# microsoft/SpeechT5

Measured on NVIDIA H100. Metric: utterances/sec (TTS fine-tune step, 10s@16kHz), higher is better.
Workload: dtype bf16

## Files before the change

### speecht5_b200/csrc/attention_flash.cu

```cuda
#include "../../include/speecht5_b200.h"
#include "kernels.cuh"
#include "ptx.cuh"
#include "tma_map.cuh"

namespace st5 {

int set_error(int code, const char* where);

constexpr int FL_T = 64;
constexpr int FL_THREADS = 9 * 32;
constexpr int FL_PE_ROWS = 128;
constexpr int FL_SP = FL_T + 4;
constexpr int FL_QPP = FL_PE_ROWS + 4;
constexpr int FL_MAX_TK_RESIDENT = 320;
constexpr int FL_MAX_T_RPE_RESIDENT = 160;
template <bool RPE> constexpr size_t fl_smem() {
  return 8192 + 2 * 8192 + 8192 + 8192 + 2 * (size_t)FL_T * FL_SP * 4 +
         (RPE ? 2 * 16384 + (size_t)FL_T * FL_QPP * 4 : 0) + 128 + 512 + 1024;
}

struct FlashFwdParams {
  int B, H, Tq, Tk, causal, maxpos;
  float scale_log2;
  const uint8_t* key_pad;
  __nv_bfloat16* out; long o_ld, o_bs;
  float* out_f32;
  float* lse; float* inv_l;
  __nv_bfloat16* psave;
  void* probs; int probs_fp32; long p_ld;
  uint32_t drop_thr; float drop_scale; uint64_t seed, offset;
  int probs_heads;
};

__device__ __forceinline__ uint32_t fl_pack(float a, float b) {
  __nv_bfloat162 t = __floats2bfloat162_rn(a, b);
  return *reinterpret_cast<uint32_t*>(&t);
}
__host__ __device__ __forceinline__ int fl_window_row0(int i0, int j0, int maxpos) {
  int w = i0 - j0 - (FL_T - 1) + maxpos;
  const int hi = 2 * maxpos - FL_PE_ROWS;
  if (w > hi) w = hi;
  if (w < 0) w = 0;
  return w;
}
template <int NR>
__device__ __forceinline__ void fl_store_acc(float* dst, int pitch, const float (&d)[NR]) {
  const int l = (int)lane_id(), w = (threadIdx.x >> 5) & 3;
  const int r0 = 16 * w + (l >> 2);
#pragma unroll
  for (int i = 0; i < NR; i += 2) {
    const int r = r0 + 8 * ((i >> 1) & 1), c = 8 * (i >> 2) + 2 * (l & 3);
    *reinterpret_cast<float2*>(dst + r * pitch + c) = make_float2(d[i], d[i + 1]);
  }
}

template <bool RPE>
__global__ void __launch_bounds__(FL_THREADS, 1)
    attn_flash_fwd_kernel(const __grid_constant__ CUtensorMap map_q, const __grid_constant__ CUtensorMap map_k,
                          const __grid_constant__ CUtensorMap map_v, const __grid_constant__ CUtensorMap map_pe,
                          const FlashFwdParams p) {
  extern __shared__ __align__(1024) uint8_t smem_raw[];
  uint8_t* smem = reinterpret_cast<uint8_t*>((reinterpret_cast<uintptr_t>(smem_raw) + 1023) & ~uintptr_t(1023));
  uint8_t* sQ = smem;
  uint8_t* sK = sQ + 8192;
  uint8_t* sV = sK + 2 * 8192;
  uint8_t* sP = sV + 8192;
  float* sS = reinterpret_cast<float*>(sP + 8192);
  float* sO = sS + FL_T * FL_SP;
  uint8_t* sPE = reinterpret_cast<uint8_t*>(sO + FL_T * FL_SP);
  float* sQP = reinterpret_cast<float*>(sPE + (RPE ? 2 * 16384 : 0));
  uint64_t* bar_q = reinterpret_cast<uint64_t*>(reinterpret_cast<uint8_t*>(sQP) + (RPE ? FL_T * FL_QPP * 4 : 0));
  uint64_t* bar_k = bar_q + 1;
  uint64_t* bar_kfree = bar_q + 3;
  uint64_t* bar_s = bar_q + 5;
  uint64_t* bar_sfree = bar_q + 6;
  uint64_t* bar_v = bar_q + 7;
  uint64_t* bar_p = bar_q + 8;
  uint64_t* bar_pv = bar_q + 9;
  uint64_t* bar_o = bar_q + 10;
  float* red = reinterpret_cast<float*>(bar_q + 16);

  const int warp = threadIdx.x >> 5;
  const int nqt = (p.Tq + FL_T - 1) / FL_T;
  const int qt = nqt - 1 - (int)blockIdx.x;
  const int h = blockIdx.y, b = blockIdx.z;
  const int i0 = qt * FL_T;
  int tk = p.Tk;
  if (p.causal && i0 + FL_T < tk) tk = i0 + FL_T;
  const int nkb = (tk + FL_T - 1) / FL_T;
  void* const probs = (p.probs_heads > 0 && h >= p.probs_heads) ? nullptr : p.probs;
  const int nsweep = probs != nullptr ? 3 : 2;
  const int NS = nsweep * nkb;

  if (warp == 4 && elect_one()) {
    tma_prefetch_desc(&map_q);
    tma_prefetch_desc(&map_k);
    tma_prefetch_desc(&map_v);
    if constexpr (RPE) tma_prefetch_desc(&map_pe);
    mbar_init(bar_q, 1);
    for (int s = 0; s < 2; ++s) {
      mbar_init(&bar_k[s], 1);
      mbar_init(&bar_kfree[s], 1);
    }
    mbar_init(bar_s, 128);
    mbar_init(bar_sfree, 4);
    mbar_init(bar_v, 1);
    mbar_init(bar_p, 4);
    mbar_init(bar_pv, 1);
    mbar_init(bar_o, 128);
    fence_mbar_init();
  }
  __syncthreads();
  pdl_sync();

  if (warp == 4) {
    if (elect_one()) {
      mbar_expect_tx(bar_q, 8192);
      tma_load_4d(sQ, &map_q, bar_q, 0, i0, h, b);
      int pv = 0;
      for (int s = 0; s < NS; ++s) {
        const int sweep = s / nkb, kb = s - sweep * nkb;
        const int st = s & 1;
        if (s >= 2) mbar_wait_quiet(&bar_kfree[st], (uint32_t)(((s >> 1) - 1) & 1));
        mbar_expect_tx(&bar_k[st], 8192u + (RPE ? 16384u : 0u));
        tma_load_4d(sK + st * 8192, &map_k, &bar_k[st], 0, kb * FL_T, h, b);
        if constexpr (RPE)
          tma_load_4d(sPE + st * 16384, &map_pe, &bar_k[st], 0, fl_window_row0(i0, kb * FL_T, p.maxpos), 0, 0);
        if (sweep == 1) {
          if (pv > 0) mbar_wait_quiet(bar_pv, (uint32_t)((pv - 1) & 1));
          mbar_expect_tx(bar_v, 8192);
          tma_load_4d(sV, &map_v, bar_v, 0, kb * FL_T, h, b);
          ++pv;
        }
      }
    }
  } else if (warp < 4) {
    mbar_wait_quiet(bar_q, 0);
    const uint32_t aq = smem_u32(sQ), ap = smem_u32(sP), av = smem_u32(sV);
    float o[32];
#pragma unroll
    for (int t = 0; t < 32; ++t) o[t] = 0.f;
    int pv = 0;
    for (int s = 0; s < NS; ++s) {
      const int sweep = s / nkb;
      const int st = s & 1;
      mbar_wait_quiet(&bar_k[st], (uint32_t)((s >> 1) & 1));
      if (s > 0) mbar_wait_quiet(bar_sfree, (uint32_t)((s - 1) & 1));
      {
        float sc[32];
        const uint32_t ak = smem_u32(sK + st * 8192);
        wgmma_fence();
#pragma unroll
        for (int k = 0; k < 4; ++k)
          wgmma_m64n64<0, 0>(sc, wgmma_smem_desc(aq + k * 32, 16, 1024), wgmma_smem_desc(ak + k * 32, 16, 1024),
                             k != 0 ? 1u : 0u);
        wgmma_commit();
        if constexpr (RPE) {
          float qp[64];
          const uint32_t ape = smem_u32(sPE + st * 16384);
#pragma unroll
          for (int k = 0; k < 4; ++k)
            wgmma_m64n128<0, 0>(qp, wgmma_smem_desc(aq + k * 32, 16, 1024), wgmma_smem_desc(ape + k * 32, 16, 1024),
                                k != 0 ? 1u : 0u);
          wgmma_commit();
          wgmma_wait<0>();
          wgmma_fence_regs(qp);
          fl_store_acc(sQP, FL_QPP, qp);
        } else {
          wgmma_wait<0>();
        }
        wgmma_fence_regs(sc);
        if (threadIdx.x == 0) mbar_arrive(&bar_kfree[st]);
        fl_store_acc(sS, FL_SP, sc);
      }
      mbar_arrive(bar_s);
      if (sweep == 1) {
        mbar_wait_quiet(bar_v, (uint32_t)(pv & 1));
        mbar_wait_quiet(bar_p, (uint32_t)(pv & 1));
        wgmma_fence();
#pragma unroll
        for (int k = 0; k < 4; ++k)
          wgmma_m64n64<0, 1>(o, wgmma_smem_desc(ap + k * 32, 16, 1024), wgmma_smem_desc(av + k * 2048, 8192, 1024),
                             (pv | k) != 0 ? 1u : 0u);
        wgmma_commit();
        wgmma_wait<0>();
        wgmma_fence_regs(o);
        if (threadIdx.x == 0) mbar_arrive(bar_pv);
        ++pv;
      }
    }
    fl_store_acc(sO, FL_SP, o);
    mbar_arrive(bar_o);
  } else {
    const int sw = warp - 5;
    const int q = sw & 1;
    const int half = sw >> 1;
    const int lane = (int)lane_id();
    const int r = q * 32 + lane;
    const int i = i0 + r;
    const bool row_ok = i < p.Tq;
    const bool warp_live = i0 + q * 32 < p.Tq;
    const uint8_t* kp = p.key_pad != nullptr ? p.key_pad + (int64_t)b * p.Tk : nullptr;
    const int64_t prow = ((int64_t)b * p.H + h) * p.Tq + i;
    uint64_t dseed = p.seed, doffset = p.offset;
    if (p.drop_thr != 0) resolve_seed(dseed, doffset);
    float* probs_f = reinterpret_cast<float*>(probs);
    __nv_bfloat16* probs_h = reinterpret_cast<__nv_bfloat16*>(probs);

    float m = -INFINITY, mm = 0.f, sum = 0.f, inv = 0.f;
    int pv = 0;
    for (int sweep = 0; sweep < nsweep; ++sweep) {
      for (int kb = 0; kb < nkb; ++kb) {
        const int s = sweep * nkb + kb;
        const int j0 = kb * FL_T;
        mbar_wait_quiet(bar_s, (uint32_t)(s & 1));
        if (sweep == 1 && pv > 0) mbar_wait_quiet(bar_pv, (uint32_t)((pv - 1) & 1));
        const int c = half;
        const int jc = j0 + c * 32;
        const bool live = warp_live && jc < tk && !(p.causal && jc > i0 + q * 32 + 31);
        uint8_t* blk = sP + r * 128;
        const int cbase = c * 4;
        if (!live) {
          if (sweep == 1) {
#pragma unroll
            for (int g = 0; g < 4; ++g) {
              *reinterpret_cast<uint4*>(blk + (((cbase + g) ^ (r & 7)) << 4)) = make_uint4(0u, 0u, 0u, 0u);
              if (p.psave != nullptr && row_ok && jc + 8 * g + 8 <= p.p_ld)
                *reinterpret_cast<uint4*>(p.psave + prow * p.p_ld + jc + 8 * g) = make_uint4(0u, 0u, 0u, 0u);
            }
          } else if (sweep == 2 && row_ok) {
            for (int t = 0; t < 32; ++t)
              if (jc + t < p.p_ld) {
                if (p.probs_fp32) probs_f[prow * p.p_ld + jc + t] = 0.f;
                else probs_h[prow * p.p_ld + jc + t] = __float2bfloat16(0.f);
              }
          }
        } else {
          float v[32];
          {
            const float* src = sS + r * FL_SP + c * 32;
#pragma unroll
            for (int t = 0; t < 32; t += 4) {
              const float4 f = *reinterpret_cast<const float4*>(src + t);
              v[t] = f.x; v[t + 1] = f.y; v[t + 2] = f.z; v[t + 3] = f.w;
            }
          }
          uint32_t vb;
          {
            const int j = jc + lane;
            const bool ok = j < tk && !(kp != nullptr && kp[j] != 0);
            vb = __ballot_sync(0xffffffffu, ok);
            if (p.causal) {
              const int lim = i - jc;
              vb &= lim >= 31 ? 0xffffffffu : (lim < 0 ? 0u : ((2u << lim) - 1u));
            }
          }
          if constexpr (RPE) {
            const int w0 = fl_window_row0(i0, j0, p.maxpos);
            int colmax = 2 * p.maxpos - 1 - w0;
            if (colmax > FL_PE_ROWS - 1) colmax = FL_PE_ROWS - 1;
            const int off = i - jc + p.maxpos - w0;
            const float* qrow = sQP + r * FL_QPP;
#pragma unroll
            for (int t = 0; t < 32; ++t) {
              int col = off - t;
              col = col < 0 ? 0 : (col > colmax ? colmax : col);
              v[t] += qrow[col];
            }
          }
          if (sweep == 0) {
#pragma unroll
            for (int t = 0; t < 32; ++t)
              if ((vb >> t) & 1u) m = fmaxf(m, v[t] * p.scale_log2);
          } else if (sweep == 1) {
            uint32_t kb_ = 0xffffffffu;
            if (p.drop_thr != 0)
              kb_ = dropout_keep_mask32(dseed, doffset, (uint64_t)prow * attn_drop_pitch(p.Tk) + (uint64_t)jc, p.drop_thr);
            __nv_bfloat16* psv = (p.psave != nullptr && row_ok) ? p.psave + prow * p.p_ld + jc : nullptr;
#pragma unroll
            for (int g = 0; g < 4; ++g) {
              float ev[8];
#pragma unroll
              for (int t = 0; t < 8; ++t) {
                const int u = 8 * g + t;
                ev[t] = ((vb >> u) & 1u) ? fast_ex2(v[u] * p.scale_log2 - mm) : 0.f;
                sum += ev[t];
              }
              const uint32_t k8 = kb_ >> (8 * g);
              uint4 pk, ps;
              pk.x = fl_pack((k8 & 1u) ? ev[0] * p.drop_scale : 0.f, (k8 & 2u) ? ev[1] * p.drop_scale : 0.f);
              pk.y = fl_pack((k8 & 4u) ? ev[2] * p.drop_scale : 0.f, (k8 & 8u) ? ev[3] * p.drop_scale : 0.f);
              pk.z = fl_pack((k8 & 16u) ? ev[4] * p.drop_scale : 0.f, (k8 & 32u) ? ev[5] * p.drop_scale : 0.f);
              pk.w = fl_pack((k8 & 64u) ? ev[6] * p.drop_scale : 0.f, (k8 & 128u) ? ev[7] * p.drop_scale : 0.f);
              *reinterpret_cast<uint4*>(blk + (((cbase + g) ^ (r & 7)) << 4)) = pk;
              if (psv != nullptr && jc + 8 * g + 8 <= p.p_ld) {
                ps.x = fl_pack((k8 & 1u) ? ev[0] : -ev[0], (k8 & 2u) ? ev[1] : -ev[1]);
                ps.y = fl_pack((k8 & 4u) ? ev[2] : -ev[2], (k8 & 8u) ? ev[3] : -ev[3]);
                ps.z = fl_pack((k8 & 16u) ? ev[4] : -ev[4], (k8 & 32u) ? ev[5] : -ev[5]);
                ps.w = fl_pack((k8 & 64u) ? ev[6] : -ev[6], (k8 & 128u) ? ev[7] : -ev[7]);
                *reinterpret_cast<uint4*>(psv + 8 * g) = ps;
              }
            }
          } else if (row_ok) {
            if (p.probs_fp32) {
              float* dst = probs_f + prow * p.p_ld + jc;
              if (jc + 32 <= p.p_ld && (p.p_ld & 3) == 0) {
#pragma unroll
                for (int t = 0; t < 32; t += 4) {
                  float4 o4;
                  o4.x = ((vb >> t) & 1u) ? fast_ex2(v[t] * p.scale_log2 - mm) * inv : 0.f;
                  o4.y = ((vb >> (t + 1)) & 1u) ? fast_ex2(v[t + 1] * p.scale_log2 - mm) * inv : 0.f;
                  o4.z = ((vb >> (t + 2)) & 1u) ? fast_ex2(v[t + 2] * p.scale_log2 - mm) * inv : 0.f;
                  o4.w = ((vb >> (t + 3)) & 1u) ? fast_ex2(v[t + 3] * p.scale_log2 - mm) * inv : 0.f;
                  *reinterpret_cast<float4*>(dst + t) = o4;
                }
              } else {
#pragma unroll
                for (int t = 0; t < 32; ++t)
                  if (jc + t < p.p_ld) dst[t] = ((vb >> t) & 1u) ? fast_ex2(v[t] * p.scale_log2 - mm) * inv : 0.f;
              }
            } else {
              __nv_bfloat16* dst = probs_h + prow * p.p_ld + jc;
#pragma unroll
              for (int t = 0; t < 32; ++t)
                if (jc + t < p.p_ld)
                  dst[t] = __float2bfloat16(((vb >> t) & 1u) ? fast_ex2(v[t] * p.scale_log2 - mm) * inv : 0.f);
            }
          }
        }
        if (sweep == 1) {
          fence_proxy_async();
          __syncwarp();
          if (lane == 0) mbar_arrive(bar_p);
          ++pv;
        }
        __syncwarp();
        if (lane == 0) mbar_arrive(bar_sfree);
      }
      if (sweep == 0) {
        red[half * FL_T + r] = m;
        asm volatile("bar.sync 1, 128;" ::: "memory");
        m = fmaxf(red[r], red[FL_T + r]);
        mm = m == -INFINITY ? 0.f : m;
        asm volatile("bar.sync 1, 128;" ::: "memory");
      } else if (sweep == 1) {
        red[half * FL_T + r] = sum;
        asm volatile("bar.sync 1, 128;" ::: "memory");
        sum = red[r] + red[FL_T + r];
        inv = sum > 0.f ? 1.f / sum : 0.f;
        if (half == 0 && row_ok) {
          if (p.lse != nullptr) p.lse[prow] = sum > 0.f ? (mm + log2f(sum)) * 0.6931471805599453f : -INFINITY;
          if (p.inv_l != nullptr) p.inv_l[prow] = inv;
        }
        asm volatile("bar.sync 1, 128;" ::: "memory");
      } else if (p.causal && half == 0 && row_ok) {
        for (int j = nkb * FL_T; j < (int)p.p_ld; ++j) {
          if (p.probs_fp32) probs_f[prow * p.p_ld + j] = 0.f;
          else probs_h[prow * p.p_ld + j] = __float2bfloat16(0.f);
        }
      }
    }
    mbar_wait_quiet(bar_o, 0);
    if (row_ok) {
      float v[32];
      const float* src = sO + r * FL_SP + half * 32;
#pragma unroll
      for (int t = 0; t < 32; t += 4) {
        const float4 f = *reinterpret_cast<const float4*>(src + t);
        v[t] = f.x * inv; v[t + 1] = f.y * inv; v[t + 2] = f.z * inv; v[t + 3] = f.w * inv;
      }
      if (p.out_f32 != nullptr) {
        float* d32 = p.out_f32 + ((int64_t)b * p.Tq + i) * (p.H * 64) + h * 64 + half * 32;
#pragma unroll
        for (int t = 0; t < 32; t += 4) *reinterpret_cast<float4*>(d32 + t) = make_float4(v[t], v[t + 1], v[t + 2], v[t + 3]);
      }
      __nv_bfloat16* dst = p.out + (int64_t)b * p.o_bs + (int64_t)i * p.o_ld + h * 64 + half * 32;
#pragma unroll
      for (int t = 0; t < 32; t += 8) {
        uint4 pk;
        pk.x = fl_pack(v[t], v[t + 1]);
        pk.y = fl_pack(v[t + 2], v[t + 3]);
        pk.z = fl_pack(v[t + 4], v[t + 5]);
        pk.w = fl_pack(v[t + 6], v[t + 7]);
        *reinterpret_cast<uint4*>(dst + t) = pk;
      }
    }
  }
}

static int fl_make_map(CUtensorMap* m, const void* ptr, int64_t rows, int64_t ld, int64_t bs, int H, int B) {
  const uint64_t dims[4] = {64, (uint64_t)rows, (uint64_t)H, (uint64_t)B};
  const uint64_t strides[3] = {(uint64_t)ld * 2, 128, (uint64_t)bs * 2};
  const uint32_t box[4] = {64, FL_T, 1, 1};
  return encode_bf16_map_4d(m, ptr, dims, strides, box);
}

static int fl_launch(const st5_attn_args* a, float* lse, void* psave, float* inv_l, float* out_f32, void* stream,
                     const char* who) {
  const bool rpe = a->pe_k != nullptr;
  CUtensorMap mq, mk, mv;
  int rc = fl_make_map(&mq, a->q, a->Tq, a->q_ld, a->q_bs, a->H, a->B);
  if (!rc) rc = fl_make_map(&mk, a->k, a->Tk, a->k_ld, a->k_bs, a->H, a->B);
  if (!rc) rc = fl_make_map(&mv, a->v, a->Tk, a->v_ld, a->v_bs, a->H, a->B);
  CUtensorMap mpe = mq;
  if (!rc && rpe) {
    const uint64_t dims[4] = {64, (uint64_t)(2 * a->maxpos), 1, 1};
    const uint64_t strides[3] = {128, (uint64_t)(2 * a->maxpos) * 128, (uint64_t)(2 * a->maxpos) * 128};
    const uint32_t box[4] = {64, FL_PE_ROWS, 1, 1};
    rc = encode_bf16_map_4d(&mpe, a->pe_k, dims, strides, box);
  }
  if (rc) return set_error(rc, who);
  static bool attr_set = false;
  if (!attr_set) {
    cudaError_t e = cudaFuncSetAttribute(attn_flash_fwd_kernel<false>, cudaFuncAttributeMaxDynamicSharedMemorySize,
                                         (int)fl_smem<false>());
    if (e == cudaSuccess)
      e = cudaFuncSetAttribute(attn_flash_fwd_kernel<true>, cudaFuncAttributeMaxDynamicSharedMemorySize,
                               (int)fl_smem<true>());
    if (e != cudaSuccess) return set_error((int)e, who);
    attr_set = true;
  }
  FlashFwdParams p;
  p.B = a->B; p.H = a->H; p.Tq = a->Tq; p.Tk = a->Tk; p.causal = a->causal; p.maxpos = a->maxpos;
  p.scale_log2 = a->scale * 1.4426950408889634f;
  p.key_pad = a->key_pad;
  p.out = (__nv_bfloat16*)a->out; p.o_ld = a->o_ld; p.o_bs = a->o_bs;
  p.out_f32 = out_f32;
  p.lse = lse; p.inv_l = inv_l;
  p.psave = reinterpret_cast<__nv_bfloat16*>(psave);
  p.probs = a->probs; p.probs_fp32 = a->probs_dtype == ST5_F32; p.p_ld = a->p_ld;
  p.probs_heads = a->probs_heads;
  p.drop_thr = drop_threshold(a->drop_p);
  p.drop_scale = a->drop_p > 0.f ? 1.f / (1.f - a->drop_p) : 1.f;
  p.seed = a->seed; p.offset = a->offset;
  dim3 grid((a->Tq + FL_T - 1) / FL_T, a->H, a->B);
  if (rpe)
    launch_pdl(attn_flash_fwd_kernel<true>, grid, dim3(FL_THREADS), fl_smem<true>(), (cudaStream_t)stream, mq, mk, mv, mpe, p);
  else
    launch_pdl(attn_flash_fwd_kernel<false>, grid, dim3(FL_THREADS), fl_smem<false>(), (cudaStream_t)stream, mq, mk, mv, mpe, p);
  return set_error((int)cudaGetLastError(), who);
}

static int fl_check_common(const st5_attn_args* a, void* psave, const float* inv_l, const char* who) {
  if ((a->probs != nullptr || psave != nullptr) && a->p_ld < a->Tk) return set_error(-3, who);
  if (psave != nullptr && ((a->p_ld & 7) || (reinterpret_cast<uintptr_t>(psave) & 15) || inv_l == nullptr))
    return set_error(-3, "attention forward: psave needs a row pitch that is a multiple of 8, 16-byte alignment and inv_l");
  if ((a->o_ld & 7) || (a->o_bs & 7) || (reinterpret_cast<uintptr_t>(a->out) & 15))
    return set_error(-4, "attention forward: out must be 16-byte aligned");
  return 0;
}

}

using namespace st5;

extern "C" int st5_attn_fused_fwd(const st5_attn_args* a, float* lse, void* psave, float* inv_l, float* out_f32,
                                  void* stream) {
  const bool rpe = a->pe_k != nullptr;
  if (a->dtype != ST5_BF16 || a->Tk > FL_MAX_TK_RESIDENT || a->Tk <= 0 || a->Tq <= 0)
    return set_error(-2, "st5_attn_fused_fwd: needs bf16 and Tk <= 320");
  if (rpe && (a->causal || a->maxpos <= 0 || a->maxpos > FL_MAX_T_RPE_RESIDENT || a->Tk > a->maxpos || a->Tq > a->maxpos))
    return set_error(-5, "st5_attn_fused_fwd: relative positions need Tq, Tk <= maxpos <= 160 (no clipping), no causal mask");
  const int rc = fl_check_common(a, psave, inv_l, "st5_attn_fused_fwd");
  if (rc) return rc;
  return fl_launch(a, lse, psave, inv_l, out_f32, stream, "st5_attn_fused_fwd");
}

extern "C" int st5_attn_flash_fwd(const st5_attn_args* a, float* lse, void* psave, float* inv_l, float* out_f32,
                                  void* stream) {
  const bool rpe = a->pe_k != nullptr;
  if (a->dtype != ST5_BF16 || a->Tk <= 0 || a->Tq <= 0) return set_error(-2, "st5_attn_flash_fwd: needs bf16");
  if (rpe && (a->causal || a->maxpos <= 0)) return set_error(-5, "st5_attn_flash_fwd: relative positions take no causal mask");
  if (a->probs != nullptr && a->probs_dtype != ST5_F32)
    return set_error(-3, "st5_attn_flash_fwd: returned probabilities are fp32");
  const int rc = fl_check_common(a, psave, inv_l, "st5_attn_flash_fwd");
  if (rc) return rc;
  return fl_launch(a, lse, psave, inv_l, out_f32, stream, "st5_attn_flash_fwd");
}
```

### speecht5_b200/csrc/ptx.cuh

```cuda
#pragma once
#include <cuda_runtime.h>
#include <cuda_bf16.h>
#include <stdint.h>
#include <stdio.h>

namespace st5 {

__device__ __forceinline__ uint32_t smem_u32(const void* p) {
  return static_cast<uint32_t>(__cvta_generic_to_shared(p));
}
__device__ __forceinline__ uint32_t lane_id() { return threadIdx.x & 31; }

__device__ __forceinline__ bool elect_one() {
  uint32_t pred = 0;
  asm volatile(
      "{\n"
      ".reg .b32 rx;\n"
      ".reg .pred px;\n"
      "elect.sync rx|px, 0xffffffff;\n"
      "selp.u32 %0, 1, 0, px;\n"
      "}\n"
      : "=r"(pred));
  return pred != 0;
}
// ... 75 lines not shown
               : "l"(map), "r"(smem_u32(src)), "r"(c0), "r"(c1), "r"(c2), "r"(c3)
               : "memory");
}
__device__ __forceinline__ void bulk_commit() { asm volatile("cp.async.bulk.commit_group;" ::: "memory"); }
__device__ __forceinline__ void bulk_wait_read0() { asm volatile("cp.async.bulk.wait_group.read 0;" ::: "memory"); }

__device__ __forceinline__ void wgmma_fence() { asm volatile("wgmma.fence.sync.aligned;" ::: "memory"); }
__device__ __forceinline__ void wgmma_commit() { asm volatile("wgmma.commit_group.sync.aligned;" ::: "memory"); }
template <int N>
__device__ __forceinline__ void wgmma_wait() { asm volatile("wgmma.wait_group.sync.aligned %0;" ::"n"(N) : "memory"); }
template <int NR>
__device__ __forceinline__ void wgmma_fence_regs(float (&d)[NR]) {
#pragma unroll
  for (int i = 0; i < NR; ++i) asm volatile("" : "+f"(d[i])::"memory");
}

template <int TA, int TB>
__device__ __forceinline__ void wgmma_m64n64(float (&d)[32], uint64_t desc_a, uint64_t desc_b, uint32_t scale_d) {
  asm volatile(
      "{\n"
      ".reg .pred p;\n"
      "setp.ne.b32 p, %34, 0;\n"
      "wgmma.mma_async.sync.aligned.m64n64k16.f32.bf16.bf16 "
      "{%0, %1, %2, %3, %4, %5, %6, %7, %8, %9, %10, %11, %12, %13, %14, %15, %16, %17, %18, %19, %20, %21, %22, %23, %24, %25, %26, %27, %28, %29, %30, %31}, "
      "%32, %33, p, 1, 1, %35, %36;\n"
      "}\n"
      : "+f"(d[0]), "+f"(d[1]), "+f"(d[2]), "+f"(d[3]), "+f"(d[4]), "+f"(d[5]), "+f"(d[6]), "+f"(d[7]),
        "+f"(d[8]), "+f"(d[9]), "+f"(d[10]), "+f"(d[11]), "+f"(d[12]), "+f"(d[13]), "+f"(d[14]), "+f"(d[15]),
        "+f"(d[16]), "+f"(d[17]), "+f"(d[18]), "+f"(d[19]), "+f"(d[20]), "+f"(d[21]), "+f"(d[22]), "+f"(d[23]),
        "+f"(d[24]), "+f"(d[25]), "+f"(d[26]), "+f"(d[27]), "+f"(d[28]), "+f"(d[29]), "+f"(d[30]), "+f"(d[31])
      : "l"(desc_a), "l"(desc_b), "r"(scale_d), "n"(TA), "n"(TB));
}

template <int TA, int TB>
__device__ __forceinline__ void wgmma_m64n128(float (&d)[64], uint64_t desc_a, uint64_t desc_b, uint32_t scale_d) {
  asm volatile(
      "{\n"
      ".reg .pred p;\n"
      "setp.ne.b32 p, %66, 0;\n"
      "wgmma.mma_async.sync.aligned.m64n128k16.f32.bf16.bf16 "
      "{%0, %1, %2, %3, %4, %5, %6, %7, %8, %9, %10, %11, %12, %13, %14, %15, %16, %17, %18, %19, %20, %21, %22, %23, %24, %25, %26, %27, %28, %29, %30, %31, %32, %33, %34, %35, %36, %37, %38, %39, %40, %41, %42, %43, %44, %45, %46, %47, %48, %49, %50, %51, %52, %53, %54, %55, %56, %57, %58, %59, %60, %61, %62, %63}, "
      "%64, %65, p, 1, 1, %67, %68;\n"
      "}\n"
      : "+f"(d[0]), "+f"(d[1]), "+f"(d[2]), "+f"(d[3]), "+f"(d[4]), "+f"(d[5]), "+f"(d[6]), "+f"(d[7]),
        "+f"(d[8]), "+f"(d[9]), "+f"(d[10]), "+f"(d[11]), "+f"(d[12]), "+f"(d[13]), "+f"(d[14]), "+f"(d[15]),
        "+f"(d[16]), "+f"(d[17]), "+f"(d[18]), "+f"(d[19]), "+f"(d[20]), "+f"(d[21]), "+f"(d[22]), "+f"(d[23]),
        "+f"(d[24]), "+f"(d[25]), "+f"(d[26]), "+f"(d[27]), "+f"(d[28]), "+f"(d[29]), "+f"(d[30]), "+f"(d[31]),
        "+f"(d[32]), "+f"(d[33]), "+f"(d[34]), "+f"(d[35]), "+f"(d[36]), "+f"(d[37]), "+f"(d[38]), "+f"(d[39]),
        "+f"(d[40]), "+f"(d[41]), "+f"(d[42]), "+f"(d[43]), "+f"(d[44]), "+f"(d[45]), "+f"(d[46]), "+f"(d[47]),
        "+f"(d[48]), "+f"(d[49]), "+f"(d[50]), "+f"(d[51]), "+f"(d[52]), "+f"(d[53]), "+f"(d[54]), "+f"(d[55]),
        "+f"(d[56]), "+f"(d[57]), "+f"(d[58]), "+f"(d[59]), "+f"(d[60]), "+f"(d[61]), "+f"(d[62]), "+f"(d[63])
      : "l"(desc_a), "l"(desc_b), "r"(scale_d), "n"(TA), "n"(TB));
}


__host__ __device__ __forceinline__ uint64_t wgmma_smem_desc(uint32_t saddr, uint32_t lbo_bytes, uint32_t sbo_bytes) {
  uint64_t d = 0;
  d |= (uint64_t)((saddr & 0x3FFFF) >> 4);
  d |= (uint64_t)((lbo_bytes >> 4) & 0x3FFF) << 16;
  d |= (uint64_t)((sbo_bytes >> 4) & 0x3FFF) << 32;
  d |= (uint64_t)1 << 62;
  return d;
}

constexpr int PHILOX_ROUNDS = 7;
struct Philox4 {
  uint32_t x, y, z, w;
};
__host__ __device__ __forceinline__ uint32_t mulhi32(uint32_t a, uint32_t b) {
  return (uint32_t)(((uint64_t)a * (uint64_t)b) >> 32);
}
__host__ __device__ __forceinline__ Philox4 philox4x32(uint64_t seed, uint64_t offset, uint64_t idx) {
  uint32_t k0 = (uint32_t)seed, k1 = (uint32_t)(seed >> 32);
  uint32_t c0 = (uint32_t)idx, c1 = (uint32_t)(idx >> 32), c2 = (uint32_t)offset, c3 = (uint32_t)(offset >> 32);
#pragma unroll
  for (int i = 0; i < PHILOX_ROUNDS; ++i) {
    uint32_t h0 = mulhi32(0xD2511F53u, c0), l0 = 0xD2511F53u * c0;
    uint32_t h1 = mulhi32(0xCD9E8D57u, c2), l1 = 0xCD9E8D57u * c2;
    uint32_t n0 = h1 ^ c1 ^ k0, n1 = l1, n2 = h0 ^ c3 ^ k1, n3 = l0;
    c0 = n0; c1 = n1; c2 = n2; c3 = n3;
    k0 += 0x9E3779B9u; k1 += 0xBB67AE85u;
  }
  return Philox4{c0, c1, c2, c3};
}
constexpr uint64_t SEED_PTR_FLAG = 1ull << 63;
__device__ __forceinline__ void resolve_seed(uint64_t& seed, uint64_t& offset) {
  if (offset & SEED_PTR_FLAG) {
    seed = *reinterpret_cast<const uint64_t*>(seed);
    offset &= ~SEED_PTR_FLAG;
  }
}
__host__ __device__ __forceinline__ uint32_t philox_lane16(const Philox4& r, int lane) {
  const uint32_t w = (lane >> 1) == 0 ? r.x : (lane >> 1) == 1 ? r.y : (lane >> 1) == 2 ? r.z : r.w;
  return (lane & 1) ? (w >> 16) : (w & 0xFFFFu);
}
__host__ __device__ __forceinline__ bool dropout_keep(uint64_t seed, uint64_t offset, uint64_t i, uint32_t thr) {
  const Philox4 r = philox4x32(seed, offset, i >> 3);
  return philox_lane16(r, (int)(i & 7)) >= thr;
}
__host__ __device__ __forceinline__ uint64_t attn_drop_pitch(int Tk) { return (uint64_t)((Tk + 31) & ~31); }
__device__ __forceinline__ uint32_t dropout_keep_mask32(uint64_t seed, uint64_t offset, uint64_t e0, uint32_t thr) {
  uint32_t mask = 0;
  const int lead = (int)((8 - (e0 & 7)) & 7);
  if (lead != 0) {
    const Philox4 r = philox4x32(seed, offset, e0 >> 3);
    for (int t = 0; t < lead; ++t)
      if (philox_lane16(r, (int)((e0 + t) & 7)) >= thr) mask |= 1u << t;
// ... 28 lines not shown
```

Baseline: 1042.

## Restructure flash attention forward into two consumer warpgroups with register-resident softmax

Rewrites the attention forward kernel so that two MMA warpgroups each own a query tile. Causal grids pair complementary tiles for load balance, and non-causal grids pair adjacent tiles. Softmax, masking and dropout now run directly on the wgmma accumulator registers, and P is fed to the PV product as a register operand. This removes the separate softmax warps, the smem round-trips for S, P and O, and the many mbarrier handshakes. K and V share a multi-stage TMA ring, with 3 stages when RPE is off. The risks are higher register pressure, duplicated QK work when probs need a third sweep, and a redundant wait on blocks past the causal limit for the shorter tile.

```diff
diff --git a/speecht5_b200/csrc/attention_flash.cu b/speecht5_b200/csrc/attention_flash.cu
--- a/speecht5_b200/csrc/attention_flash.cu
+++ b/speecht5_b200/csrc/attention_flash.cu
@@ -10,13 +10,14 @@
 constexpr int FL_T = 64;
 constexpr int FL_THREADS = 9 * 32;
 constexpr int FL_PE_ROWS = 128;
-constexpr int FL_SP = FL_T + 4;
 constexpr int FL_QPP = FL_PE_ROWS + 4;
 constexpr int FL_MAX_TK_RESIDENT = 320;
 constexpr int FL_MAX_T_RPE_RESIDENT = 160;
+template <bool RPE> constexpr int fl_stages() { return RPE ? 2 : 3; }
+template <bool RPE> constexpr uint32_t fl_stage_bytes() { return 2 * 8192 + (RPE ? 2 * 16384 : 0); }
 template <bool RPE> constexpr size_t fl_smem() {
-  return 8192 + 2 * 8192 + 8192 + 8192 + 2 * (size_t)FL_T * FL_SP * 4 +
-         (RPE ? 2 * 16384 + (size_t)FL_T * FL_QPP * 4 : 0) + 128 + 512 + 1024;
+  return 2 * 8192 + (size_t)fl_stages<RPE>() * fl_stage_bytes<RPE>() + (RPE ? 2 * (size_t)FL_T * FL_QPP * 4 : 0) +
+         128 + 1024;
 }
 
 struct FlashFwdParams {
@@ -43,6 +44,20 @@
   if (w < 0) w = 0;
   return w;
 }
+__device__ __forceinline__ void fl_tiles(int x, int nqt, bool causal, int& ta, int& tb) {
+  if (causal) {
+    ta = nqt - 1 - x;
+    tb = x < ta ? x : -1;
+  } else {
+    ta = 2 * x;
+    tb = 2 * x + 1 < nqt ? 2 * x + 1 : -1;
+  }
+}
+__device__ __forceinline__ int fl_tile_nkb(int t, int Tk, bool causal) {
+  int tk = Tk;
+  if (causal && (t + 1) * FL_T < tk) tk = (t + 1) * FL_T;
+  return (tk + FL_T - 1) / FL_T;
+}
 template <int NR>
 __device__ __forceinline__ void fl_store_acc(float* dst, int pitch, const float (&d)[NR]) {
   const int l = (int)lane_id(), w = (threadIdx.x >> 5) & 3;
@@ -52,6 +67,40 @@
     const int r = r0 + 8 * ((i >> 1) & 1), c = 8 * (i >> 2) + 2 * (l & 3);
     *reinterpret_cast<float2*>(dst + r * pitch + c) = make_float2(d[i], d[i + 1]);
   }
+}
+__device__ __forceinline__ void fl_bar_wg(int id) { asm volatile("bar.sync %0, 128;" ::"r"(id) : "memory"); }
+__device__ __forceinline__ void fl_fence_u32(uint32_t (&a)[4][4]) {
+#pragma unroll
+  for (int k = 0; k < 4; ++k)
+#pragma unroll
+    for (int i = 0; i < 4; ++i) asm volatile("" : "+r"(a[k][i])::"memory");
+}
+__device__ __forceinline__ uint32_t fl_keep_bits(uint64_t seed, uint64_t offset, uint64_t e0, uint64_t e1,
+                                                 uint32_t thr) {
+  const int lane = (int)lane_id(), qd = lane & 3;
+  uint32_t mine = 0;
+#pragma unroll
+  for (int ri = 0; ri < 2; ++ri)
+#pragma unroll
+    for (int cc = 0; cc < 2; ++cc) {
+      const Philox4 r = philox4x32(seed, offset, ((ri ? e1 : e0) + 16 * qd + 8 * cc) >> 3);
+#pragma unroll
+      for (int l = 0; l < 8; ++l)
+        if (philox_lane16(r, l) >= thr) mine |= 1u << (8 * (2 * ri + cc) + l);
+    }
+  uint32_t keep = 0;
+#pragma unroll
+  for (int src = 0; src < 4; ++src) {
+    const uint32_t x = __shfl_sync(0xffffffffu, mine, (lane & ~3) | src);
+#pragma unroll
+    for (int cc = 0; cc < 2; ++cc)
+#pragma unroll
+      for (int ri = 0; ri < 2; ++ri) {
+        const uint32_t bits = (x >> (8 * (2 * ri + cc) + 2 * qd)) & 3u;
+        keep |= bits << (4 * (2 * src + cc) + 2 * ri);
+      }
+  }
+  return keep;
 }
 
 template <bool RPE>
@@ -59,331 +108,254 @@
     attn_flash_fwd_kernel(const __grid_constant__ CUtensorMap map_q, const __grid_constant__ CUtensorMap map_k,
                           const __grid_constant__ CUtensorMap map_v, const __grid_constant__ CUtensorMap map_pe,
                           const FlashFwdParams p) {
+  constexpr int ST = fl_stages<RPE>();
+  constexpr uint32_t SB = fl_stage_bytes<RPE>();
   extern __shared__ __align__(1024) uint8_t smem_raw[];
   uint8_t* smem = reinterpret_cast<uint8_t*>((reinterpret_cast<uintptr_t>(smem_raw) + 1023) & ~uintptr_t(1023));
   uint8_t* sQ = smem;
-  uint8_t* sK = sQ + 8192;
-  uint8_t* sV = sK + 2 * 8192;
-  uint8_t* sP = sV + 8192;
-  float* sS = reinterpret_cast<float*>(sP + 8192);
-  float* sO = sS + FL_T * FL_SP;
-  uint8_t* sPE = reinterpret_cast<uint8_t*>(sO + FL_T * FL_SP);
-  float* sQP = reinterpret_cast<float*>(sPE + (RPE ? 2 * 16384 : 0));
-  uint64_t* bar_q = reinterpret_cast<uint64_t*>(reinterpret_cast<uint8_t*>(sQP) + (RPE ? FL_T * FL_QPP * 4 : 0));
-  uint64_t* bar_k = bar_q + 1;
-  uint64_t* bar_kfree = bar_q + 3;
-  uint64_t* bar_s = bar_q + 5;
-  uint64_t* bar_sfree = bar_q + 6;
-  uint64_t* bar_v = bar_q + 7;
-  uint64_t* bar_p = bar_q + 8;
-  uint64_t* bar_pv = bar_q + 9;
-  uint64_t* bar_o = bar_q + 10;
-  float* red = reinterpret_cast<float*>(bar_q + 16);
+  uint8_t* sStage = sQ + 2 * 8192;
+  float* sQP = reinterpret_cast<float*>(sStage + ST * SB);
+  uint64_t* bar_q = reinterpret_cast<uint64_t*>(reinterpret_cast<uint8_t*>(sQP) + (RPE ? 2 * FL_T * FL_QPP * 4 : 0));
+  uint64_t* bar_full = bar_q + 1;
+  uint64_t* bar_free = bar_full + ST;
 
   const int warp = threadIdx.x >> 5;
   const int nqt = (p.Tq + FL_T - 1) / FL_T;
-  const int qt = nqt - 1 - (int)blockIdx.x;
+  int ta, tb;
+  fl_tiles((int)blockIdx.x, nqt, p.causal != 0, ta, tb);
+  const int nwg = tb >= 0 ? 2 : 1;
   const int h = blockIdx.y, b = blockIdx.z;
-  const int i0 = qt * FL_T;
-  int tk = p.Tk;
-  if (p.causal && i0 + FL_T < tk) tk = i0 + FL_T;
-  const int nkb = (tk + FL_T - 1) / FL_T;
+  const int nkbm = fl_tile_nkb(ta, p.Tk, p.causal != 0);
   void* const probs = (p.probs_heads > 0 && h >= p.probs_heads) ? nullptr : p.probs;
   const int nsweep = probs != nullptr ? 3 : 2;
-  const int NS = nsweep * nkb;
-
-  if (warp == 4 && elect_one()) {
+
+  if (warp == 8 && elect_one()) {
     tma_prefetch_desc(&map_q);
     tma_prefetch_desc(&map_k);
     tma_prefetch_desc(&map_v);
     if constexpr (RPE) tma_prefetch_desc(&map_pe);
     mbar_init(bar_q, 1);
-    for (int s = 0; s < 2; ++s) {
-      mbar_init(&bar_k[s], 1);
-      mbar_init(&bar_kfree[s], 1);
-    }
-    mbar_init(bar_s, 128);
-    mbar_init(bar_sfree, 4);
-    mbar_init(bar_v, 1);
-    mbar_init(bar_p, 4);
-    mbar_init(bar_pv, 1);
-    mbar_init(bar_o, 128);
+    for (int s = 0; s < ST; ++s) {
+      mbar_init(&bar_full[s], 1);
+      mbar_init(&bar_free[s], nwg);
+    }
     fence_mbar_init();
   }
   __syncthreads();
   pdl_sync();
 
-  if (warp == 4) {
+  if (warp == 8) {
     if (elect_one()) {
-      mbar_expect_tx(bar_q, 8192);
-      tma_load_4d(sQ, &map_q, bar_q, 0, i0, h, b);
-      int pv = 0;
+      mbar_expect_tx(bar_q, 8192u * nwg);
+      tma_load_4d(sQ, &map_q, bar_q, 0, ta * FL_T, h, b);
+      if (tb >= 0) tma_load_4d(sQ + 8192, &map_q, bar_q, 0, tb * FL_T, h, b);
+      const int NS = nsweep * nkbm;
       for (int s = 0; s < NS; ++s) {
-        const int sweep = s / nkb, kb = s - sweep * nkb;
-        const int st = s & 1;
-        if (s >= 2) mbar_wait_quiet(&bar_kfree[st], (uint32_t)(((s >> 1) - 1) & 1));
-        mbar_expect_tx(&bar_k[st], 8192u + (RPE ? 16384u : 0u));
-        tma_load_4d(sK + st * 8192, &map_k, &bar_k[st], 0, kb * FL_T, h, b);
-        if constexpr (RPE)
-          tma_load_4d(sPE + st * 16384, &map_pe, &bar_k[st], 0, fl_window_row0(i0, kb * FL_T, p.maxpos), 0, 0);
-        if (sweep == 1) {
-          if (pv > 0) mbar_wait_quiet(bar_pv, (uint32_t)((pv - 1) & 1));
-          mbar_expect_tx(bar_v, 8192);
-          tma_load_4d(sV, &map_v, bar_v, 0, kb * FL_T, h, b);
-          ++pv;
-        }
-      }
-    }
-  } else if (warp < 4) {
-    mbar_wait_quiet(bar_q, 0);
-    const uint32_t aq = smem_u32(sQ), ap = smem_u32(sP), av = smem_u32(sV);
-    float o[32];
-#pragma unroll
-    for (int t = 0; t < 32; ++t) o[t] = 0.f;
-    int pv = 0;
-    for (int s = 0; s < NS; ++s) {
-      const int sweep = s / nkb;
-      const int st = s & 1;
-      mbar_wait_quiet(&bar_k[st], (uint32_t)((s >> 1) & 1));
-      if (s > 0) mbar_wait_quiet(bar_sfree, (uint32_t)((s - 1) & 1));
+        const int sweep = s / nkbm, kb = s - sweep * nkbm, st = s % ST;
+        if (s >= ST) mbar_wait_quiet(&bar_free[st], (uint32_t)((s / ST - 1) & 1));
+        uint8_t* stg = sStage + st * SB;
+        mbar_expect_tx(&bar_full[st], (sweep == 1 ? 16384u : 8192u) + (RPE ? 16384u * nwg : 0u));
+        tma_load_4d(stg, &map_k, &bar_full[st], 0, kb * FL_T, h, b);
+        if (sweep == 1) tma_load_4d(stg + 8192, &map_v, &bar_full[st], 0, kb * FL_T, h, b);
+        if constexpr (RPE) {
+          tma_load_4d(stg + 16384, &map_pe, &bar_full[st], 0, fl_window_row0(ta * FL_T, kb * FL_T, p.maxpos), 0, 0);
+          if (tb >= 0)
+            tma_load_4d(stg + 32768, &map_pe, &bar_full[st], 0, fl_window_row0(tb * FL_T, kb * FL_T, p.maxpos), 0, 0);
+        }
+      }
+    }
+    return;
+  }
+
+  const int wg = warp >> 2, wl = warp & 3;
+  const int t = wg == 0 ? ta : tb;
+  if (t < 0) return;
+  const bool lead = (threadIdx.x & 127) == 0;
+  const int i0 = t * FL_T;
+  int tk = p.Tk;
+  if (p.causal && i0 + FL_T < tk) tk = i0 + FL_T;
+  const int nkb = (tk + FL_T - 1) / FL_T;
+  const int lane = (int)lane_id(), qd = lane & 3;
+  const int r0 = 16 * wl + (lane >> 2);
+  const bool row_ok[2] = {i0 + r0 < p.Tq, i0 + r0 + 8 < p.Tq};
+  const int64_t prow0 = ((int64_t)b * p.H + h) * p.Tq + i0 + r0;
+  const int rh = i0 + 32 * (wl >> 1);
+  const uint8_t* kp = p.key_pad != nullptr ? p.key_pad + (int64_t)b * p.Tk : nullptr;
+  uint64_t dseed = p.seed, doffset = p.offset;
+  if (p.drop_thr != 0) resolve_seed(dseed, doffset);
+  const uint64_t dpitch = attn_drop_pitch(p.Tk);
+  float* probs_f = reinterpret_cast<float*>(probs);
+  __nv_bfloat16* probs_h = reinterpret_cast<__nv_bfloat16*>(probs);
+  const uint32_t aq = smem_u32(sQ + wg * 8192);
+  float* qpw = sQP + wg * FL_T * FL_QPP;
+
+  float o[32];
+#pragma unroll
+  for (int i = 0; i < 32; ++i) o[i] = 0.f;
+  float m[2] = {-INFINITY, -INFINITY}, mm[2] = {0.f, 0.f}, sum[2] = {0.f, 0.f}, inv[2] = {0.f, 0.f};
+  mbar_wait_quiet(bar_q, 0);
+  for (int sweep = 0; sweep < nsweep; ++sweep) {
+    for (int kb = 0; kb < nkbm; ++kb) {
+      const int s = sweep * nkbm + kb, st = s % ST;
+      mbar_wait_quiet(&bar_full[st], (uint32_t)((s / ST) & 1));
+      if (kb >= nkb) {
+        if (lead) mbar_arrive(&bar_free[st]);
+        continue;
+      }
+      const int j0 = kb * FL_T;
+      const uint32_t astg = smem_u32(sStage + st * SB);
+      uint32_t vm = 0;
+      bool live[2];
       {
-        float sc[32];
-        const uint32_t ak = smem_u32(sK + st * 8192);
+        const int ja = j0 + lane, jb = j0 + 32 + lane;
+        const uint32_t oka = __ballot_sync(0xffffffffu, ja < p.Tk && !(kp != nullptr && kp[ja] != 0));
+        const uint32_t okb = __ballot_sync(0xffffffffu, jb < p.Tk && !(kp != nullptr && kp[jb] != 0));
+#pragma unroll
+        for (int ch = 0; ch < 2; ++ch) {
+          const int jc = j0 + 32 * ch;
+          live[ch] = rh < p.Tq && jc < tk && !(p.causal && jc > rh + 31);
+        }
+        const uint64_t okk = (live[0] ? (uint64_t)oka : 0ull) | (live[1] ? (uint64_t)okb << 32 : 0ull);
+#pragma unroll
+        for (int ri = 0; ri < 2; ++ri) {
+          uint64_t rm = okk;
+          if (p.causal) {
+            const int lim = i0 + r0 + 8 * ri - j0;
+            rm &= lim >= 63 ? ~0ull : (lim < 0 ? 0ull : (2ull << lim) - 1ull);
+          }
+          const uint32_t lo = (uint32_t)(rm >> (2 * qd)), hi = (uint32_t)(rm >> (32 + 2 * qd));
+#pragma unroll
+          for (int c = 0; c < 8; ++c)
+            vm |= (((c < 4 ? lo : hi) >> (8 * (c & 3))) & 3u) << (4 * c + 2 * ri);
+        }
+      }
+      uint32_t keep = 0xffffffffu;
+      if (sweep == 1 && p.drop_thr != 0)
+        keep = fl_keep_bits(dseed, doffset, (uint64_t)prow0 * dpitch + j0, (uint64_t)(prow0 + 8) * dpitch + j0,
+                            p.drop_thr);
+      if constexpr (RPE) {
+        float qp[64];
+        const uint32_t ape = astg + 16384 + wg * 16384;
         wgmma_fence();
 #pragma unroll
         for (int k = 0; k < 4; ++k)
-          wgmma_m64n64<0, 0>(sc, wgmma_smem_desc(aq + k * 32, 16, 1024), wgmma_smem_desc(ak + k * 32, 16, 1024),
-                             k != 0 ? 1u : 0u);
+          wgmma_m64n128<0, 0>(qp, wgmma_smem_desc(aq + k * 32, 16, 1024), wgmma_smem_desc(ape + k * 32, 16, 1024),
+                              k != 0 ? 1u : 0u);
         wgmma_commit();
-        if constexpr (RPE) {
-          float qp[64];
-          const uint32_t ape = smem_u32(sPE + st * 16384);
-#pragma unroll
-          for (int k = 0; k < 4; ++k)
-            wgmma_m64n128<0, 0>(qp, wgmma_smem_desc(aq + k * 32, 16, 1024), wgmma_smem_desc(ape + k * 32, 16, 1024),
-                                k != 0 ? 1u : 0u);
-          wgmma_commit();
-          wgmma_wait<0>();
-          wgmma_fence_regs(qp);
-          fl_store_acc(sQP, FL_QPP, qp);
-        } else {
-          wgmma_wait<0>();
-        }
-        wgmma_fence_regs(sc);
-        if (threadIdx.x == 0) mbar_arrive(&bar_kfree[st]);
-        fl_store_acc(sS, FL_SP, sc);
-      }
-      mbar_arrive(bar_s);
-      if (sweep == 1) {
-        mbar_wait_quiet(bar_v, (uint32_t)(pv & 1));
-        mbar_wait_quiet(bar_p, (uint32_t)(pv & 1));
+        wgmma_wait<0>();
+        wgmma_fence_regs(qp);
+        fl_bar_wg(1 + wg);
+        fl_store_acc(qpw, FL_QPP, qp);
+      }
+      float sc[32];
+      wgmma_fence();
+#pragma unroll
+      for (int k = 0; k < 4; ++k)
+        wgmma_m64n64<0, 0>(sc, wgmma_smem_desc(aq + k * 32, 16, 1024), wgmma_smem_desc(astg + k * 32, 16, 1024),
+                           k != 0 ? 1u : 0u);
+      wgmma_commit();
+      if constexpr (RPE) fl_bar_wg(1 + wg);
+      wgmma_wait<0>();
+      wgmma_fence_regs(sc);
+      if (sweep != 1 && lead) mbar_arrive(&bar_free[st]);
+      if constexpr (RPE) {
+        const int w0 = fl_window_row0(i0, j0, p.maxpos);
+        int colmax = 2 * p.maxpos - 1 - w0;
+        if (colmax > FL_PE_ROWS - 1) colmax = FL_PE_ROWS - 1;
+        const int off = i0 + r0 - j0 - 2 * qd + p.maxpos - w0;
+        const float* qrow = qpw + r0 * FL_QPP;
+#pragma unroll
+        for (int i = 0; i < 32; ++i) {
+          const int ri = (i >> 1) & 1;
+          int col = off + 8 * ri - 8 * (i >> 2) - (i & 1);
+          col = col < 0 ? 0 : (col > colmax ? colmax : col);
+          sc[i] += qrow[8 * ri * FL_QPP + col];
+        }
+      }
+      if (sweep == 0) {
+#pragma unroll
+        for (int i = 0; i < 32; ++i)
+          if ((vm >> i) & 1u) m[(i >> 1) & 1] = fmaxf(m[(i >> 1) & 1], sc[i] * p.scale_log2);
+      } else if (sweep == 1) {
+        uint32_t pa[4][4];
+#pragma unroll
+        for (int i = 0; i < 32; i += 2) {
+          const int ri = (i >> 1) & 1, c = i >> 2;
+          const float e0 = ((vm >> i) & 1u) ? fast_ex2(sc[i] * p.scale_log2 - mm[ri]) : 0.f;
+          const float e1 = ((vm >> (i + 1)) & 1u) ? fast_ex2(sc[i + 1] * p.scale_log2 - mm[ri]) : 0.f;
+          sum[ri] += e0;
+          sum[ri] += e1;
+          const bool k0 = (keep >> i) & 1u, k1 = (keep >> (i + 1)) & 1u;
+          pa[c >> 1][(c & 1) << 1 | ri] =
+              fl_pack(k0 ? e0 * p.drop_scale : 0.f, k1 ? e1 * p.drop_scale : 0.f);
+          const int jcol = j0 + 8 * c;
+          if (p.psave != nullptr && row_ok[ri] && jcol + 8 <= p.p_ld)
+            *reinterpret_cast<uint32_t*>(p.psave + (prow0 + 8 * ri) * p.p_ld + jcol + 2 * qd) =
+                live[c >> 2] ? fl_pack(k0 ? e0 : -e0, k1 ? e1 : -e1) : 0u;
+        }
+        const uint32_t av = astg + 8192;
         wgmma_fence();
 #pragma unroll
         for (int k = 0; k < 4; ++k)
-          wgmma_m64n64<0, 1>(o, wgmma_smem_desc(ap + k * 32, 16, 1024), wgmma_smem_desc(av + k * 2048, 8192, 1024),
-                             (pv | k) != 0 ? 1u : 0u);
+          wgmma_m64n64_rs<1>(o, pa[k], wgmma_smem_desc(av + k * 2048, 8192, 1024), 1u);
         wgmma_commit();
         wgmma_wait<0>();
         wgmma_fence_regs(o);
-        if (threadIdx.x == 0) mbar_arrive(bar_pv);
-        ++pv;
-      }
-    }
-    fl_store_acc(sO, FL_SP, o);
-    mbar_arrive(bar_o);
-  } else {
-    const int sw = warp - 5;
-    const int q = sw & 1;
-    const int half = sw >> 1;
-    const int lane = (int)lane_id();
-    const int r = q * 32 + lane;
-    const int i = i0 + r;
-    const bool row_ok = i < p.Tq;
-    const bool warp_live = i0 + q * 32 < p.Tq;
-    const uint8_t* kp = p.key_pad != nullptr ? p.key_pad + (int64_t)b * p.Tk : nullptr;
-    const int64_t prow = ((int64_t)b * p.H + h) * p.Tq + i;
-    uint64_t dseed = p.seed, doffset = p.offset;
-    if (p.drop_thr != 0) resolve_seed(dseed, doffset);
-    float* probs_f = reinterpret_cast<float*>(probs);
-    __nv_bfloat16* probs_h = reinterpret_cast<__nv_bfloat16*>(probs);
-
-    float m = -INFINITY, mm = 0.f, sum = 0.f, inv = 0.f;
-    int pv = 0;
-    for (int sweep = 0; sweep < nsweep; ++sweep) {
-      for (int kb = 0; kb < nkb; ++kb) {
-        const int s = sweep * nkb + kb;
-        const int j0 = kb * FL_T;
-        mbar_wait_quiet(bar_s, (uint32_t)(s & 1));
-        if (sweep == 1 && pv > 0) mbar_wait_quiet(bar_pv, (uint32_t)((pv - 1) & 1));
-        const int c = half;
-        const int jc = j0 + c * 32;
-        const bool live = warp_live && jc < tk && !(p.causal && jc > i0 + q * 32 + 31);
-        uint8_t* blk = sP + r * 128;
-        const int cbase = c * 4;
-        if (!live) {
-          if (sweep == 1) {
-#pragma unroll
-            for (int g = 0; g < 4; ++g) {
-              *reinterpret_cast<uint4*>(blk + (((cbase + g) ^ (r & 7)) << 4)) = make_uint4(0u, 0u, 0u, 0u);
-              if (p.psave != nullptr && row_ok && jc + 8 * g + 8 <= p.p_ld)
-                *reinterpret_cast<uint4*>(p.psave + prow * p.p_ld + jc + 8 * g) = make_uint4(0u, 0u, 0u, 0u);
-            }
-          } else if (sweep == 2 && row_ok) {
-            for (int t = 0; t < 32; ++t)
-              if (jc + t < p.p_ld) {
-                if (p.probs_fp32) probs_f[prow * p.p_ld + jc + t] = 0.f;
-                else probs_h[prow * p.p_ld + jc + t] = __float2bfloat16(0.f);
-              }
+        fl_fence_u32(pa);
+        if (lead) mbar_arrive(&bar_free[st]);
+      } else {
+#pragma unroll
+        for (int i = 0; i < 32; ++i) {
+          const int ri = (i >> 1) & 1;
+          const int j = j0 + 8 * (i >> 2) + 2 * qd + (i & 1);
+          if (row_ok[ri] && j < p.p_ld) {
+            const float pr = ((vm >> i) & 1u) ? fast_ex2(sc[i] * p.scale_log2 - mm[ri]) * inv[ri] : 0.f;
+            if (p.probs_fp32) probs_f[(prow0 + 8 * ri) * p.p_ld + j] = pr;
+            else probs_h[(prow0 + 8 * ri) * p.p_ld + j] = __float2bfloat16(pr);
           }
-        } else {
-          float v[32];
-          {
-            const float* src = sS + r * FL_SP + c * 32;
-#pragma unroll
-            for (int t = 0; t < 32; t += 4) {
-              const float4 f = *reinterpret_cast<const float4*>(src + t);
-              v[t] = f.x; v[t + 1] = f.y; v[t + 2] = f.z; v[t + 3] = f.w;
-            }
+        }
+      }
+    }
+    if (sweep == 0) {
+#pragma unroll
+      for (int ri = 0; ri < 2; ++ri) {
+        m[ri] = fmaxf(m[ri], __shfl_xor_sync(0xffffffffu, m[ri], 1));
+        m[ri] = fmaxf(m[ri], __shfl_xor_sync(0xffffffffu, m[ri], 2));
+        mm[ri] = m[ri] == -INFINITY ? 0.f : m[ri];
+      }
+    } else if (sweep == 1) {
+#pragma unroll
+      for (int ri = 0; ri < 2; ++ri) {
+        sum[ri] += __shfl_xor_sync(0xffffffffu, sum[ri], 1);
+        sum[ri] += __shfl_xor_sync(0xffffffffu, sum[ri], 2);
+        inv[ri] = sum[ri] > 0.f ? 1.f / sum[ri] : 0.f;
+        if (qd == 0 && row_ok[ri]) {
+          const int64_t pr = prow0 + 8 * ri;
+          if (p.lse != nullptr) p.lse[pr] = sum[ri] > 0.f ? (mm[ri] + log2f(sum[ri])) * 0.6931471805599453f : -INFINITY;
+          if (p.inv_l != nullptr) p.inv_l[pr] = inv[ri];
+        }
+      }
+    } else if (p.causal) {
+#pragma unroll
+      for (int ri = 0; ri < 2; ++ri)
+        if (row_ok[ri])
+          for (int j = nkb * FL_T + qd; j < (int)p.p_ld; j += 4) {
+            if (p.probs_fp32) probs_f[(prow0 + 8 * ri) * p.p_ld + j] = 0.f;
+            else probs_h[(prow0 + 8 * ri) * p.p_ld + j] = __float2bfloat16(0.f);
           }
-          uint32_t vb;
-          {
-            const int j = jc + lane;
-            const bool ok = j < tk && !(kp != nullptr && kp[j] != 0);
-            vb = __ballot_sync(0xffffffffu, ok);
-            if (p.causal) {
-              const int lim = i - jc;
-              vb &= lim >= 31 ? 0xffffffffu : (lim < 0 ? 0u : ((2u << lim) - 1u));
-            }
-          }
-          if constexpr (RPE) {
-            const int w0 = fl_window_row0(i0, j0, p.maxpos);
-            int colmax = 2 * p.maxpos - 1 - w0;
-            if (colmax > FL_PE_ROWS - 1) colmax = FL_PE_ROWS - 1;
-            const int off = i - jc + p.maxpos - w0;
-            const float* qrow = sQP + r * FL_QPP;
-#pragma unroll
-            for (int t = 0; t < 32; ++t) {
-              int col = off - t;
-              col = col < 0 ? 0 : (col > colmax ? colmax : col);
-              v[t] += qrow[col];
-            }
-          }
-          if (sweep == 0) {
-#pragma unroll
-            for (int t = 0; t < 32; ++t)
-              if ((vb >> t) & 1u) m = fmaxf(m, v[t] * p.scale_log2);
-          } else if (sweep == 1) {
-            uint32_t kb_ = 0xffffffffu;
-            if (p.drop_thr != 0)
-              kb_ = dropout_keep_mask32(dseed, doffset, (uint64_t)prow * attn_drop_pitch(p.Tk) + (uint64_t)jc, p.drop_thr);
-            __nv_bfloat16* psv = (p.psave != nullptr && row_ok) ? p.psave + prow * p.p_ld + jc : nullptr;
-#pragma unroll
-            for (int g = 0; g < 4; ++g) {
-              float ev[8];
-#pragma unroll
-              for (int t = 0; t < 8; ++t) {
-                const int u = 8 * g + t;
-                ev[t] = ((vb >> u) & 1u) ? fast_ex2(v[u] * p.scale_log2 - mm) : 0.f;
-                sum += ev[t];
-              }
-              const uint32_t k8 = kb_ >> (8 * g);
-              uint4 pk, ps;
-              pk.x = fl_pack((k8 & 1u) ? ev[0] * p.drop_scale : 0.f, (k8 & 2u) ? ev[1] * p.drop_scale : 0.f);
-              pk.y = fl_pack((k8 & 4u) ? ev[2] * p.drop_scale : 0.f, (k8 & 8u) ? ev[3] * p.drop_scale : 0.f);
-              pk.z = fl_pack((k8 & 16u) ? ev[4] * p.drop_scale : 0.f, (k8 & 32u) ? ev[5] * p.drop_scale : 0.f);
-              pk.w = fl_pack((k8 & 64u) ? ev[6] * p.drop_scale : 0.f, (k8 & 128u) ? ev[7] * p.drop_scale : 0.f);
-              *reinterpret_cast<uint4*>(blk + (((cbase + g) ^ (r & 7)) << 4)) = pk;
-              if (psv != nullptr && jc + 8 * g + 8 <= p.p_ld) {
-                ps.x = fl_pack((k8 & 1u) ? ev[0] : -ev[0], (k8 & 2u) ? ev[1] : -ev[1]);
-                ps.y = fl_pack((k8 & 4u) ? ev[2] : -ev[2], (k8 & 8u) ? ev[3] : -ev[3]);
-                ps.z = fl_pack((k8 & 16u) ? ev[4] : -ev[4], (k8 & 32u) ? ev[5] : -ev[5]);
-                ps.w = fl_pack((k8 & 64u) ? ev[6] : -ev[6], (k8 & 128u) ? ev[7] : -ev[7]);
-                *reinterpret_cast<uint4*>(psv + 8 * g) = ps;
-              }
-            }
-          } else if (row_ok) {
-            if (p.probs_fp32) {
-              float* dst = probs_f + prow * p.p_ld + jc;
-              if (jc + 32 <= p.p_ld && (p.p_ld & 3) == 0) {
-#pragma unroll
-                for (int t = 0; t < 32; t += 4) {
-                  float4 o4;
-                  o4.x = ((vb >> t) & 1u) ? fast_ex2(v[t] * p.scale_log2 - mm) * inv : 0.f;
-                  o4.y = ((vb >> (t + 1)) & 1u) ? fast_ex2(v[t + 1] * p.scale_log2 - mm) * inv : 0.f;
-                  o4.z = ((vb >> (t + 2)) & 1u) ? fast_ex2(v[t + 2] * p.scale_log2 - mm) * inv : 0.f;
-                  o4.w = ((vb >> (t + 3)) & 1u) ? fast_ex2(v[t + 3] * p.scale_log2 - mm) * inv : 0.f;
-                  *reinterpret_cast<float4*>(dst + t) = o4;
-                }
-              } else {
-#pragma unroll
-                for (int t = 0; t < 32; ++t)
-                  if (jc + t < p.p_ld) dst[t] = ((vb >> t) & 1u) ? fast_ex2(v[t] * p.scale_log2 - mm) * inv : 0.f;
-              }
-            } else {
-              __nv_bfloat16* dst = probs_h + prow * p.p_ld + jc;
-#pragma unroll
-              for (int t = 0; t < 32; ++t)
-                if (jc + t < p.p_ld)
-                  dst[t] = __float2bfloat16(((vb >> t) & 1u) ? fast_ex2(v[t] * p.scale_log2 - mm) * inv : 0.f);
-            }
-          }
-        }
-        if (sweep == 1) {
-          fence_proxy_async();
-          __syncwarp();
-          if (lane == 0) mbar_arrive(bar_p);
-          ++pv;
-        }
-        __syncwarp();
-        if (lane == 0) mbar_arrive(bar_sfree);
-      }
-      if (sweep == 0) {
-        red[half * FL_T + r] = m;
-        asm volatile("bar.sync 1, 128;" ::: "memory");
-        m = fmaxf(red[r], red[FL_T + r]);
-        mm = m == -INFINITY ? 0.f : m;
-        asm volatile("bar.sync 1, 128;" ::: "memory");
-      } else if (sweep == 1) {
-        red[half * FL_T + r] = sum;
-        asm volatile("bar.sync 1, 128;" ::: "memory");
-        sum = red[r] + red[FL_T + r];
-        inv = sum > 0.f ? 1.f / sum : 0.f;
-        if (half == 0 && row_ok) {
-          if (p.lse != nullptr) p.lse[prow] = sum > 0.f ? (mm + log2f(sum)) * 0.6931471805599453f : -INFINITY;
-          if (p.inv_l != nullptr) p.inv_l[prow] = inv;
-        }
-        asm volatile("bar.sync 1, 128;" ::: "memory");
-      } else if (p.causal && half == 0 && row_ok) {
-        for (int j = nkb * FL_T; j < (int)p.p_ld; ++j) {
-          if (p.probs_fp32) probs_f[prow * p.p_ld + j] = 0.f;
-          else probs_h[prow * p.p_ld + j] = __float2bfloat16(0.f);
-        }
-      }
-    }
-    mbar_wait_quiet(bar_o, 0);
-    if (row_ok) {
-      float v[32];
-      const float* src = sO + r * FL_SP + half * 32;
-#pragma unroll
-      for (int t = 0; t < 32; t += 4) {
-        const float4 f = *reinterpret_cast<const float4*>(src + t);
-        v[t] = f.x * inv; v[t + 1] = f.y * inv; v[t + 2] = f.z * inv; v[t + 3] = f.w * inv;
-      }
-      if (p.out_f32 != nullptr) {
-        float* d32 = p.out_f32 + ((int64_t)b * p.Tq + i) * (p.H * 64) + h * 64 + half * 32;
-#pragma unroll
-        for (int t = 0; t < 32; t += 4) *reinterpret_cast<float4*>(d32 + t) = make_float4(v[t], v[t + 1], v[t + 2], v[t + 3]);
-      }
-      __nv_bfloat16* dst = p.out + (int64_t)b * p.o_bs + (int64_t)i * p.o_ld + h * 64 + half * 32;
-#pragma unroll
-      for (int t = 0; t < 32; t += 8) {
-        uint4 pk;
-        pk.x = fl_pack(v[t], v[t + 1]);
-        pk.y = fl_pack(v[t + 2], v[t + 3]);
-        pk.z = fl_pack(v[t + 4], v[t + 5]);
-        pk.w = fl_pack(v[t + 6], v[t + 7]);
-        *reinterpret_cast<uint4*>(dst + t) = pk;
-      }
+    }
+  }
+#pragma unroll
+  for (int ri = 0; ri < 2; ++ri) {
+    if (!row_ok[ri]) continue;
+    const int i = i0 + r0 + 8 * ri;
+    float* d32 = p.out_f32 != nullptr ? p.out_f32 + ((int64_t)b * p.Tq + i) * (p.H * 64) + h * 64 + 2 * qd : nullptr;
+    __nv_bfloat16* dst = p.out + (int64_t)b * p.o_bs + (int64_t)i * p.o_ld + h * 64 + 2 * qd;
+#pragma unroll
+    for (int c = 0; c < 8; ++c) {
+      const float v0 = o[4 * c + 2 * ri] * inv[ri], v1 = o[4 * c + 2 * ri + 1] * inv[ri];
+      if (d32 != nullptr) *reinterpret_cast<float2*>(d32 + 8 * c) = make_float2(v0, v1);
+      *reinterpret_cast<uint32_t*>(dst + 8 * c) = fl_pack(v0, v1);
     }
   }
 }
@@ -433,7 +405,7 @@
   p.drop_thr = drop_threshold(a->drop_p);
   p.drop_scale = a->drop_p > 0.f ? 1.f / (1.f - a->drop_p) : 1.f;
   p.seed = a->seed; p.offset = a->offset;
-  dim3 grid((a->Tq + FL_T - 1) / FL_T, a->H, a->B);
+  dim3 grid(((a->Tq + FL_T - 1) / FL_T + 1) / 2, a->H, a->B);
   if (rpe)
     launch_pdl(attn_flash_fwd_kernel<true>, grid, dim3(FL_THREADS), fl_smem<true>(), (cudaStream_t)stream, mq, mk, mv, mpe, p);
   else
diff --git a/speecht5_b200/csrc/ptx.cuh b/speecht5_b200/csrc/ptx.cuh
--- a/speecht5_b200/csrc/ptx.cuh
+++ b/speecht5_b200/csrc/ptx.cuh
@@ -151,7 +151,23 @@
         "+f"(d[56]), "+f"(d[57]), "+f"(d[58]), "+f"(d[59]), "+f"(d[60]), "+f"(d[61]), "+f"(d[62]), "+f"(d[63])
       : "l"(desc_a), "l"(desc_b), "r"(scale_d), "n"(TA), "n"(TB));
 }
-
+template <int TB>
+__device__ __forceinline__ void wgmma_m64n64_rs(float (&d)[32], const uint32_t (&a)[4], uint64_t desc_b,
+                                                uint32_t scale_d) {
+  asm volatile(
+      "{\n"
+      ".reg .pred p;\n"
+      "setp.ne.b32 p, %37, 0;\n"
+      "wgmma.mma_async.sync.aligned.m64n64k16.f32.bf16.bf16 "
+      "{%0, %1, %2, %3, %4, %5, %6, %7, %8, %9, %10, %11, %12, %13, %14, %15, %16, %17, %18, %19, %20, %21, %22, %23, %24, %25, %26, %27, %28, %29, %30, %31}, "
+      "{%32, %33, %34, %35}, %36, p, 1, 1, %38;\n"
+      "}\n"
+      : "+f"(d[0]), "+f"(d[1]), "+f"(d[2]), "+f"(d[3]), "+f"(d[4]), "+f"(d[5]), "+f"(d[6]), "+f"(d[7]),
+        "+f"(d[8]), "+f"(d[9]), "+f"(d[10]), "+f"(d[11]), "+f"(d[12]), "+f"(d[13]), "+f"(d[14]), "+f"(d[15]),
+        "+f"(d[16]), "+f"(d[17]), "+f"(d[18]), "+f"(d[19]), "+f"(d[20]), "+f"(d[21]), "+f"(d[22]), "+f"(d[23]),
+        "+f"(d[24]), "+f"(d[25]), "+f"(d[26]), "+f"(d[27]), "+f"(d[28]), "+f"(d[29]), "+f"(d[30]), "+f"(d[31])
+      : "r"(a[0]), "r"(a[1]), "r"(a[2]), "r"(a[3]), "l"(desc_b), "r"(scale_d), "n"(TB));
+}
 
 __host__ __device__ __forceinline__ uint64_t wgmma_smem_desc(uint32_t saddr, uint32_t lbo_bytes, uint32_t sbo_bytes) {
   uint64_t d = 0;
```

Result: faster. 1075 (median of 6 runs) (+3.1%).
